# Meeso1/nmmo

Hardware: AMD Instinct MI355X
Metric: agent-steps/sec (whole node), 128-agent envs at 1/2/4/8 MI355X (higher is better)
Workload: dtype int16

## Files before the change

nmmo_amd/csrc/agent_obs.h:

```cpp
#pragma once

#include <utility>

#include "kernels.h"
#include "wire.h"

namespace nmmo {

#ifndef NMMO_AO_WAVES
#define NMMO_AO_WAVES 4
#define NMMO_AO_AGENTS 16
#endif
constexpr int kAoWaves = NMMO_AO_WAVES;
constexpr int kAoAgents = NMMO_AO_AGENTS;
constexpr int kAoRows = kMaxSlots / 64;
constexpr uint32_t kAoEmpty = 0xFFFFFFFFu;
static_assert(kSize <= 256 && kMaxSlots <= 2 * 256 && kMaxSlots % 64 == 0, "packed entity word; two slots per thread (>= 256 threads)");
__host__ __device__ inline int ao_stride(int S) { return ((S + 1) >> 1 | 1) << 1; }
__host__ __device__ inline size_t ao_entity_lds(int S) {
  return (((size_t)NMMO_N_ENTITY_COLS * ao_stride(S) * 2 + 15) & ~(size_t)15) + (size_t)(kMaxSlots + 64) * 4;
}
__host__ __device__ inline uint32_t ao_pack(int slot, int row, int col, bool immune, bool danger, bool player) {
  return (uint32_t)(row & 255) | (uint32_t)(slot & 255) << 8 | (uint32_t)(col & 255) << 16 | (uint32_t)(slot >> 8) << 24 |
         (immune ? 1u << 25 : 0u) | (danger ? 1u << 26 : 0u) | (player ? 1u << 27 : 0u);
}
__device__ __forceinline__ int ao_slot(uint32_t w) { return (int)(((w >> 8) & 255u) | ((w >> 16) & 256u)); }
__device__ __forceinline__ int ao_row(uint32_t w) { return (int)(w & 255u); }
__device__ __forceinline__ int ao_col(uint32_t w) { return (int)((w >> 16) & 255u); }
__device__ __forceinline__ bool ao_immune(uint32_t w) { return (w >> 25) & 1u; }
__device__ __forceinline__ bool ao_danger(uint32_t w) { return (w >> 26) & 1u; }
__device__ __forceinline__ bool ao_player(uint32_t w) { return (w >> 27) & 1u; }
typedef unsigned short ao_u16x2 __attribute__((ext_vector_type(2)));
__device__ __forceinline__ bool ao_in_window(uint32_t w, uint32_t rc) {
  ao_u16x2 d = __builtin_bit_cast(ao_u16x2, w & 0x00FF00FFu) - __builtin_bit_cast(ao_u16x2, rc) +
               (ao_u16x2){(unsigned short)kVision, (unsigned short)kVision};
  return (d.x > d.y ? d.x : d.y) <= 2 * kVision;
}
static_assert(kMaxSlots <= 512 && kSize <= 255, "packed entity word");

constexpr int kSecN[12] = {3, 101, NMMO_MARKET_ROWS + 1, kInv + 1, kInv + 1, kNObs + 1, 99, kNObs + 1, 5, kInv + 1, 99, kInv + 1};
__host__ __device__ constexpr int sec_flat(int k) { return k == 0 ? 0 : sec_flat(k - 1) + kSecN[k - 1]; }
__host__ __device__ constexpr int sec_wire(int k) { return k < 2 ? sec_flat(k) : sec_flat(k) - kWireBuyN; }
static_assert(sec_flat(2) == kWireBuyLo && sec_flat(12) == kMaskN && sec_flat(1) == kMkAttackT &&
                  sec_flat(3) == kMkDestroy && sec_flat(4) == kMkGiveI && sec_flat(5) == kMkGiveT &&
                  sec_flat(6) == kMkGoldP && sec_flat(7) == kMkGoldT && sec_flat(8) == kMkMove &&
                  sec_flat(9) == kMkSellI && sec_flat(10) == kMkSellP && sec_flat(11) == kMkUse,
              "sections (wire.h)");
__host__ inline bool ao_layout_ok(const ObsParams& p) {
  const int offs[12] = {p.o_style, p.o_target, p.o_buy, p.o_destroy, p.o_give_item, p.o_give_target,
                        p.o_gg_price, p.o_gg_target, p.o_move, p.o_sell_item, p.o_sell_price, p.o_use};
  for (int k = 0; k < 12; k++)
    if (offs[k] != sec_flat(k)) return false;
  return p.o_agent_id == sec_flat(12);
}

__device__ __forceinline__ int ao_lane() {
  int l = (int)(threadIdx.x & 63u);
  asm volatile("" : "+v"(l));
  return l;
}

__device__ __forceinline__ uint64_t low_bits(int n) { return n >= 64 ? ~0ull : n <= 0 ? 0ull : (1ull << n) - 1ull; }
template <int L>
__device__ __forceinline__ int writelane(int v, int x) {
  static_assert(L >= 0 && L < 64, "lane");
  int sv = __builtin_amdgcn_readfirstlane(v);
  asm volatile("" : "+s"(sv));
  asm volatile("v_writelane_b32 %0, %1, %2" : "+v"(x) : "s"(sv), "n"(L));
  return x;
}
template <int kLane0, int kIdx0, int... D>
__device__ __forceinline__ int writelanes_(const uint32_t* img, int x, std::integer_sequence<int, D...>) {
  ((x = writelane<kLane0 + D>((int)img[kIdx0 + D], x)), ...);
  return x;
}
template <int kLane0, int kIdx0, int kN>
__device__ __forceinline__ int writelanes(const uint32_t* img, int x) {
  return writelanes_<kLane0, kIdx0>(img, x, std::make_integer_sequence<int, kN>{});
}

template <int kOff, int kN, int kW>
__device__ __forceinline__ void put_field(uint32_t (&img)[kW], uint64_t lo, uint64_t hi) {
  static_assert((kOff + kN + 31) / 32 <= kW, "image size");
#pragma unroll
  for (int d = kOff / 32; d <= (kOff + kN - 1) / 32; d++) {
    const int st = 32 * d - kOff;
    uint32_t x;
    if (st < 0) x = (uint32_t)(lo << (-st));
    else if (st == 0) x = (uint32_t)lo;
    else if (st < 64) x = (uint32_t)((lo >> st) | (hi << (64 - st)));
    else x = (uint32_t)(hi >> (st - 64));
    img[d] |= x;
  }
}

constexpr int kAoStageIt = (NMMO_N_ENTITY_COLS * (kMaxSlots / 8) + 255) / 256;
struct AoStage {
  uint4 x[kAoStageIt];
  int al[2], ds[2];
  int nm, mv;
};
__device__ __forceinline__ void ao_stage_load(const ObsParams& p, int e, AoStage& r) {
  const int S = p.S, tid = threadIdx.x;
  const int16_t* E = p.ent + (size_t)e * NMMO_NF * S;
  const int w4 = S / 8;
  const int nw = NMMO_N_ENTITY_COLS * w4;
  r.nm = p.mcount[e];
  r.mv = p.mlist[(size_t)e * NMMO_MARKET_ROWS + min(tid, NMMO_MARKET_ROWS - 1)];
#pragma unroll
  for (int k = 0; k < kAoStageIt; k++) {
    const int i = tid + (int)blockDim.x * k;
    const int f = i / w4, j = i - f * w4;
    r.x[k] = i < nw ? reinterpret_cast<const uint4*>(E + (size_t)f * S)[j] : make_uint4(0u, 0u, 0u, 0u);
  }
#pragma unroll
  for (int u = 0; u < 2; u++) {
    const int s = min(tid + (int)blockDim.x * u, S - 1);
    r.al[u] = E[F_ALIVE * S + s];
    r.ds[u] = E[F_DS_ROW * S + s];
  }
}
__device__ __forceinline__ void ao_stage_store(const ObsParams& p, int e, int16_t* T, uint32_t* pk, const AoStage& r) {
  const int S = p.S, P = p.P, Sp = ao_stride(S), tid = threadIdx.x;
  const int16_t* E = p.ent + (size_t)e * NMMO_NF * S;
  const int w4 = S / 8;
  const int nw = NMMO_N_ENTITY_COLS * w4;
  constexpr int kIt = kAoStageIt;
  const int(&al)[2] = r.al;
  const int(&ds)[2] = r.ds;
#pragma unroll
  for (int k = 0; k < kIt; k++) {
    const int i = tid + (int)blockDim.x * k;
    if (i < nw) {
      const int f = i / w4, j = i - f * w4;
      uint32_t* d = reinterpret_cast<uint32_t*>(T + f * Sp) + 4 * j;
      d[0] = r.x[k].x;
      d[1] = r.x[k].y;
      d[2] = r.x[k].z;
      d[3] = r.x[k].w;
    }
  }
  for (int i = tid + (int)blockDim.x * kIt; i < nw; i += blockDim.x) {
    const int f = i / w4, j = i - f * w4;
    const uint4 y = reinterpret_cast<const uint4*>(E + (size_t)f * S)[j];
    uint32_t* d = reinterpret_cast<uint32_t*>(T + f * Sp) + 4 * j;
    d[0] = y.x;
    d[1] = y.y;
    d[2] = y.z;
    d[3] = y.w;
  }
  for (int k = tid; k < kMaxSlots + 64; k += blockDim.x) pk[k] = kAoEmpty;
  __syncthreads();
#pragma unroll
  for (int u = 0; u < 2; u++) {
    const int s = tid + (int)blockDim.x * u;
    if (s < S && al[u] && (unsigned)(ds[u] - 1) < (unsigned)S) {
      const bool player = s < P;
      const bool immune = player && T[F_TIME_ALIVE * Sp + s] < p.spawn_immunity;
      const bool danger = T[F_NPC_TYPE * Sp + s] > 1;
      pk[ds[u] - 1] = ao_pack(s, T[F_ROW * Sp + s], T[F_COL * Sp + s], immune, danger, player);
    }
  }
  __syncthreads();
}
__device__ __forceinline__ uint2 ao_listing_load(const ObsParams& p, int e, const AoStage& r) {
  const int own = min((r.mv >> 16) & 255, p.P - 1), slot = min((r.mv >> 24) & 15, kInv - 1);
  return p.items[((size_t)e * p.P + own) * kInv + slot];
}

__device__ __forceinline__ void ao_env_group(int n_envs, int G, int& e, int& g) {
  const int id = blockIdx.x;
  if ((n_envs & 7) == 0) {
    const int x = id & 7, q = id >> 3;
    g = q % G;
    e = (q / G) * 8 + x;
  } else {
    e = id / G;
    g = id - e * G;
  }
}

constexpr int kAoWinRowBytes = 20;
constexpr int kAoWinAgentBytes = 15 * kAoWinRowBytes;
__host__ __device__ inline size_t ao_win_lds(int agents = kAoAgents) {
  return (size_t)agents * kAoWinAgentBytes + (size_t)agents * kInv * 8;
}
__device__ __forceinline__ int ao_clamp_pos(int x) { return min(max(x, kVision), kSize - 1 - kVision); }
struct AoNoop {
  __device__ void operator()() const {}
};
template <int kAgents = kAoAgents, typename F = AoNoop>
__device__ inline void ao_stage_windows(const ObsParams& p, int e, int g, const int16_t* T, int Sp, uint32_t* ws, uint2* is,
                                        F before_barrier = F()) {
  const int tid = threadIdx.x, P = p.P;
  const int la = tid / 15, row = tid - 15 * la, a = g * kAgents + la;
  const bool win = tid < kAgents * 15 && a < P;
  uint32_t d[5] = {0u, 0u, 0u, 0u, 0u};
  if (win) {
    const int r = ao_clamp_pos(T[F_ROW * Sp + a]), c = ao_clamp_pos(T[F_COL * Sp + a]);
    const int base = (r - kVision + row) * kSize + c - kVision;
    const uint32_t* src = reinterpret_cast<const uint32_t*>(p.mat + (size_t)e * kTiles) + (base >> 2);
#pragma unroll
    for (int k = 0; k < 5; k++) d[k] = src[k];
  }
  uint2 iw = make_uint2(0u, 0u);
  const bool itm = tid < kAgents * kInv && g * kAgents + tid / kInv < P;
  if (itm) iw = p.items[((size_t)e * P + g * kAgents) * kInv + tid];
  if (win) {
#pragma unroll
    for (int k = 0; k < 5; k++) ws[tid * 5 + k] = d[k];
  }
  if (tid < kAgents * kInv) is[tid] = iw;
  before_barrier();
  __syncthreads();
}
__device__ __forceinline__ void ao_win_offsets(int (&wo)[2]) {
  wo[0] = wo[1] = 0;
#pragma unroll
  for (int i = 0; i < 4; i++) {
    const int t = lane_id() + 64 * i;
    const int o = t < 225 ? (t / 15) * kAoWinRowBytes + t % 15 : 0;
    wo[i >> 1] |= o << (16 * (i & 1));
  }
}
__device__ __forceinline__ int ao_win_off(const int (&wo)[2], int i) { return (wo[i >> 1] >> (16 * (i & 1))) & 0xFFFF; }

__device__ __forceinline__ int ao_compact(const uint32_t (&pr)[kAoRows], int S, int r, int c, uint32_t* visw) {
  int nvis = 0;
  const uint32_t rc = (uint32_t)r | (uint32_t)c << 16;
#pragma unroll
  for (int i = 0; i < kAoRows; i++) {
    if (64 * i >= S) break;
    const uint32_t x = pr[i];
    const bool in = ao_in_window(x, rc);
    const uint64_t b = __ballot(in);
    const int pos = nvis + __popcll(b & lanes_below());
    if (in && pos < kNObs) visw[pos] = x;
    nvis += __popcll(b);
  }
  return nvis;
}

__device__ __forceinline__ void ao_window_offsets(int (&mo)[2]) {
  mo[0] = mo[1] = 0;
#pragma unroll
  for (int i = 0; i < 4; i++) {
    const int t = lane_id() + 64 * i;
    const int o = t < 225 ? (t / 15 - kVision) * kSize + t % 15 - kVision : 0;
    mo[i >> 1] |= (o & 0xFFFF) << (16 * (i & 1));
  }
}
__device__ __forceinline__ int ao_window_off(const int (&mo)[2], int i) {
  return (int)(int16_t)(uint16_t)((uint32_t)mo[i >> 1] >> (16 * (i & 1)));
}

__device__ __forceinline__ uint32_t ao_move_bits(uint32_t wm1) {
  uint32_t b = 0u;
#pragma unroll
  for (int d = 0; d < 5; d++) {
    const int t = (kVision + dir_dr(d)) * 15 + kVision + dir_dc(d);
    if (!impassable((int)__builtin_amdgcn_readlane((int)wm1, t - 64))) b |= 1u << d;
  }
  return b;
}

static_assert(F_ALCHEMY_LEVEL == F_MELEE_LEVEL + 14 && F_FISHING_LEVEL == F_MELEE_LEVEL + 6 &&
                  F_HERBALISM_LEVEL == F_MELEE_LEVEL + 8, "skill level fields");
__host__ __device__ constexpr uint64_t ao_req_lut() {
  uint64_t m = 0;
  for (int t = 0; t < 16; t++) {
    const int k = (t >= T_SPEAR && t <= T_WAND) ? t - T_SPEAR : (t >= T_WHETSTONE && t <= T_RUNES) ? t - T_WHETSTONE
                  : (t >= T_ROD && t <= T_CHISEL) ? 3 + t - T_ROD : 8;
    m |= (uint64_t)k << (4 * t);
  }
  return m;
}
static_assert(T_RATION == 16 && T_POTION == 17, "requirement table: ration -> fishing, potion -> herbalism");
__device__ __forceinline__ uint64_t ao_usable_ballot(const int16_t* T, int Sp, int ti, uint2 it, bool have) {
  const int lane = ao_lane();
  int lv = 0;
  if (lane < 8) {
    lv = T[(F_MELEE_LEVEL + 2 * lane) * Sp + ti];
  } else if (lane == 8) {
    lv = max((int)T[F_MELEE_LEVEL * Sp + ti], max((int)T[F_RANGE_LEVEL * Sp + ti], (int)T[F_MAGE_LEVEL * Sp + ti]));
  }
  const int type = it_type(it);
  const int k = type < 16 ? (int)((ao_req_lut() >> (4 * type)) & 15u) : type == T_RATION ? 3 : type == T_POTION ? 4 : 8;
  const int req = __shfl(lv, k);
  const bool eq = type >= T_HAT && type <= T_RUNES && it_equipped(it);
  return __ballot(have && !it_price(it) && (eq || it_level(it) <= req));
}

struct AoSections {
  uint64_t s0, s1[2], s3, s4, s5[2], s6[2], s7[2], s8, s9, s10[2], s11;
};
struct AoAgent {
  int a, ti, r, c, gold, aid, nv, ninv, prev_price;
  uint32_t mv;
};
template <bool kWrap>
__device__ __forceinline__ AoSections ao_sections(const ObsParams& p, const int16_t* T, int Sp, const uint32_t* visw,
                                                 const AoAgent& g, uint2 it) {
  const bool combat = (p.systems & NMMO_SYS_COMBAT) != 0;
  const bool item = (p.systems & NMMO_SYS_ITEM) != 0;
  const bool exch = item && (p.systems & NMMO_SYS_EXCHANGE) != 0;
  const bool no_give = kWrap && (p.wflags & kWrapObsNoGive);
  const bool no_danger = kWrap && (p.wflags & kWrapObsNoDangerous);
  const int lane = ao_lane();
  AoSections x;
  x.s1[0] = x.s1[1] = x.s5[0] = x.s5[1] = x.s7[0] = x.s7[1] = 0ull;
#pragma unroll
  for (int h = 0; h < 2; h++) {
    if (64 * h >= g.nv) break;
    const int k = 64 * h + lane;
    bool tgt = false, st = false;
    if (k < g.nv) {
      const uint32_t w = visw[k];
      const int q = ao_slot(w);
      tgt = combat && q != g.a && linf(g.r, g.c, ao_row(w), ao_col(w)) <= 3 && !ao_immune(w) &&
            !(no_danger && ao_danger(w));
      st = ao_player(w) && q != g.a && ao_row(w) == g.r && ao_col(w) == g.c;
    }
    x.s1[h] = __ballot(tgt);
    const uint64_t sb = __ballot(st);
    if (item && !no_give) x.s5[h] = sb;
    if (exch && !no_give) x.s7[h] = sb;
  }
  x.s1[1] |= 1ull << (kNObs - 64);
  x.s5[1] |= 1ull << (kNObs - 64);
  x.s7[1] |= 1ull << (kNObs - 64);
  const bool have = lane < g.ninv;
  const bool fr = have && !it_equipped(it) && !it_price(it);
  const uint64_t bfr = __ballot(fr);
  x.s3 = (item ? bfr : 0ull) | 1ull << kInv;
  x.s4 = (item && !no_give ? bfr : 0ull) | 1ull << kInv;
  x.s9 = (exch ? __ballot(have && !it_equipped(it)) : 0ull) | 1ull << kInv;
  x.s11 = (item ? ao_usable_ballot(T, Sp, g.ti, it, have) : 0ull) | 1ull << kInv;
  x.s0 = combat ? low_bits(kSecN[0]) : 0ull;
  x.s6[0] = x.s6[1] = x.s10[0] = x.s10[1] = 0ull;
  if (exch) {
    const int ng = no_give ? min(g.gold, 1) : min(g.gold, kSecN[6]);
    x.s6[0] = low_bits(ng);
    x.s6[1] = low_bits(ng - 64);
    x.s10[0] = low_bits(kSecN[10]);
    x.s10[1] = low_bits(kSecN[10] - 64);
    if constexpr (kWrap) {
      const int pp = g.prev_price;
      if ((p.wflags & kWrapObsPrice) && pp >= 0 && pp < kSecN[10]) {
        const uint64_t clr = ~(1ull << (pp & 63));
        if (pp < 64) x.s10[0] &= clr;
        else x.s10[1] &= clr;
      }
    }
  }
  x.s8 = g.mv;
  return x;
}

template <bool kFlat, int kW>
__device__ __forceinline__ void ao_image(const AoSections& x, uint32_t (&img)[kW]) {
#pragma unroll
  for (int d = 0; d < kW; d++) img[d] = 0u;
#define AO_PUT(k, lo, hi) put_field<kFlat ? sec_flat(k) : sec_wire(k), kSecN[k], kW>(img, lo, hi)
  AO_PUT(0, x.s0, 0ull);
  AO_PUT(1, x.s1[0], x.s1[1]);
  AO_PUT(3, x.s3, 0ull);
  AO_PUT(4, x.s4, 0ull);
  AO_PUT(5, x.s5[0], x.s5[1]);
  AO_PUT(6, x.s6[0], x.s6[1]);
  AO_PUT(7, x.s7[0], x.s7[1]);
  AO_PUT(8, x.s8, 0ull);
  AO_PUT(9, x.s9, 0ull);
  AO_PUT(10, x.s10[0], x.s10[1]);
  AO_PUT(11, x.s11, 0ull);
#undef AO_PUT
}

}
```

nmmo_amd/csrc/flat_obs.hip:

```cpp
#include "agent_obs.h"

namespace nmmo {

#ifndef NMMO_FO_ABL
#define NMMO_FO_ABL 0
#endif
#ifndef NMMO_FO_STAMPS
#define NMMO_FO_STAMPS 0
#endif
#if NMMO_FO_STAMPS
constexpr int kFoStamps = 12;
__device__ uint64_t fo_stamp_buf[1 << 17][kFoStamps];
__device__ uint64_t fo_wave_buf[1 << 15][6];
#define FO_STAMP(k) fst[k] = __builtin_amdgcn_s_memtime()
#else
#define FO_STAMP(k) (void)0
#endif
#ifndef NMMO_FO_XCD
#define NMMO_FO_XCD 1
#endif
#ifndef NMMO_FO_TILE_SKIP
#define NMMO_FO_TILE_SKIP 0
#endif
#ifndef NMMO_FO_TASK_BATCH
#define NMMO_FO_TASK_BATCH 8
#endif
constexpr int kFoTaskBatch = NMMO_FO_TASK_BATCH;
constexpr int kFoStagedListings = 256;
constexpr int kFoChunks = 25;
static_assert(kFoChunks * 64 >= kMaskN + 2 && (kFoChunks - 1) * 64 < kMaskN, "mask chunks");
static_assert(sec_flat(2) == 104 && sec_flat(3) == 104 + NMMO_MARKET_ROWS + 1, "Buy.MarketItem bits");
constexpr int kFoBuyLo = sec_flat(2);
constexpr int kFoId = kMaskN, kFoEntity = kFoId + 2, kFoInv = kFoEntity + kNObs * NMMO_N_ENTITY_COLS,
              kFoMarket = kFoInv + kInv * 16, kFoTask = kFoMarket + NMMO_MARKET_ROWS * 16;

__host__ __device__ inline size_t fo_lds_bytes(int S) {
  return ao_entity_lds(S) + (size_t)NMMO_MARKET_ROWS * 2 + (size_t)kFoStagedListings * 8 +
         (size_t)kAoWaves * 128 * 4 + ao_win_lds();
}

template <int kSh>
__device__ __forceinline__ uint64_t fo_shift(uint64_t lo, uint64_t hi) {
  if constexpr (kSh >= 64) {
    return 0ull;
  } else if constexpr (kSh > 0) {
    return lo << kSh;
  } else if constexpr (kSh == 0) {
    return lo;
  } else if constexpr (-kSh < 64) {
    return (lo >> (-kSh)) | (hi << (64 + kSh));
  } else if constexpr (-kSh < 128) {
    return hi >> (-kSh - 64);
  } else {
    return 0ull;
  }
}
template <int kK, int kC>
__device__ __forceinline__ uint64_t fo_sec(uint64_t lo, uint64_t hi) {
  constexpr int off = sec_flat(kK), n = kSecN[kK];
  if constexpr (off >= 64 * kC + 64 || off + n <= 64 * kC) return 0ull;
  else return fo_shift<off - 64 * kC>(lo, hi);
}
template <int kC>
__device__ __forceinline__ uint64_t fo_chunk(const AoSections& x) {
  return fo_sec<0, kC>(x.s0, 0ull) | fo_sec<1, kC>(x.s1[0], x.s1[1]) | fo_sec<3, kC>(x.s3, 0ull) |
         fo_sec<4, kC>(x.s4, 0ull) | fo_sec<5, kC>(x.s5[0], x.s5[1]) | fo_sec<6, kC>(x.s6[0], x.s6[1]) |
         fo_sec<7, kC>(x.s7[0], x.s7[1]) | fo_sec<8, kC>(x.s8, 0ull) | fo_sec<9, kC>(x.s9, 0ull) |
         fo_sec<10, kC>(x.s10[0], x.s10[1]) | fo_sec<11, kC>(x.s11, 0ull);
}
__device__ __forceinline__ float fo_bit(uint64_t m) { return __builtin_amdgcn_inverse_ballot_w64(m) ? 1.f : 0.f; }
__device__ __forceinline__ void fo_st(float* row, uint32_t idx, float v) {
  *reinterpret_cast<float*>(reinterpret_cast<char*>(row) + (idx << 2)) = v;
}

constexpr int kFoTail0 = (kFoBuyLo + NMMO_MARKET_ROWS) / 64;
__host__ __device__ constexpr int fo_slot(int c) { return c < 2 ? c : c - kFoTail0 + 2; }
static_assert(fo_slot(kFoChunks - 1) == 9 && kZext == 10 + 1 + 12, "tracked chunks | position | items");
struct FoImg {
  bool ext;
  uint32_t lo, hi;
  int j10;
  int nimg;
  int nst;
};
__device__ __forceinline__ uint64_t fo_prev(const FoImg& g, int slot) {
  return (uint64_t)(uint32_t)__builtin_amdgcn_readlane((int)g.lo, g.j10 + slot) |
         (uint64_t)(uint32_t)__builtin_amdgcn_readlane((int)g.hi, g.j10 + slot) << 32;
}
template <int kC>
__device__ __forceinline__ void fo_put(float* row, FoImg& g, uint64_t m, float aid, float tick) {
  constexpr int sl = fo_slot(kC);
  const int lane = ao_lane();
  const bool same = g.ext && m == fo_prev(g, sl);
  if constexpr (kC == kFoChunks - 1) {
    constexpr int n = kMaskN - 64 * kC;
    if (!same) {
      if (lane < n + 2) fo_st(row, 64 * kC + lane, lane < n ? fo_bit(m) : lane == n ? aid : tick);
      g.nst += n + 2;
    } else {
      if (lane == n + 1) fo_st(row, 64 * kC + lane, tick);
      g.nst += 1;
    }
  } else if (!same) {
    fo_st(row, 64 * kC + lane, fo_bit(m));
    g.nst += 64;
  }
  g.nimg = writelane<2 * sl>((int)(uint32_t)m, g.nimg);
  g.nimg = writelane<2 * sl + 1>((int)(uint32_t)(m >> 32), g.nimg);
}
template <int kC>
__device__ __forceinline__ void fo_tail_chunks(float* row, FoImg& g, const AoSections& x, uint64_t buy17, float aid,
                                               float tick) {
  if constexpr (kC < kFoChunks) {
    uint64_t m = fo_chunk<kC>(x);
    if constexpr (kC == kFoTail0) m |= buy17 | 1ull << ((kFoBuyLo + NMMO_MARKET_ROWS) & 63);
    fo_put<kC>(row, g, m, aid, tick);
    fo_tail_chunks<kC + 1>(row, g, x, buy17, aid, tick);
  }
}

struct IcDesc {
  uint32_t tmA, tmB;
  uint32_t f;
};
__device__ __forceinline__ IcDesc ic_desc(int col) {
  auto bits = [](int lo, int hi) { return ((2u << hi) - 1u) & ~((1u << lo) - 1u); };
  IcDesc d{0u, 0u, 0u};
  auto bf = [&](int sel, int sh, int wd) { d.f = (uint32_t)(sel | sh << 1 | wd << 6); };
  switch (col) {
    case 0: bf(1, 16, 16); break;
    case 1: bf(0, 0, 5); break;
    case 2: d.f = 1u << 11; break;
    case 3: bf(0, 5, 4); break;
    case 5: bf(1, 0, 16); break;
    case 6: case 7: case 8:
      d.tmA = 1u << (T_SPEAR + col - 6) | 1u << (T_WHETSTONE + col - 6);
      d.f = 5u << 12 | 5u << 20;
      break;
    case 9: case 10: case 11:
      d.tmA = bits(T_HAT, T_BOTTOM);
      d.tmB = bits(T_ROD, T_CHISEL);
      d.f = 3u << 12 | 2u << 16;
      break;
    case 12: d.tmA = 1u << T_POTION; d.f = 5u << 12 | 50u << 20; break;
    case 13: d.tmA = 1u << T_RATION; d.f = 5u << 12 | 50u << 20; break;
    case 14: bf(0, 9, 1); break;
    case 15: bf(0, 10, 7); break;
    default: break;
  }
  return d;
}
__device__ __forceinline__ float ic_value(uint2 w, int owner, const IcDesc& d) {
  const int type = (int)(w.x & 31u), lvl = (int)((w.x >> 5) & 15u);
  const uint32_t bfv = __builtin_amdgcn_ubfe((d.f & 1u) ? w.y : w.x, (d.f >> 1) & 31u, (d.f >> 6) & 31u);
  const int ta = (int)((d.tmA >> type) & 1u), tb = (int)((d.tmB >> type) & 1u);
  const int mult = ta * (int)((d.f >> 12) & 15u) + tb * (int)((d.f >> 16) & 15u);
  return (float)((int)bfv + (int)((d.f >> 11) & 1u) * owner + mult * lvl + ((ta | tb) ? (int)(d.f >> 20) : 0));
}
static_assert(T_POTION < 32 && T_RATION < 32 && T_WHETSTONE + 2 < 32, "item type masks");

__device__ __forceinline__ int fo_compact(const uint32_t (&pr)[kAoRows], int r, int c, uint32_t* visw) {
  int nvis = 0;
  const uint32_t rc = (uint32_t)r | (uint32_t)c << 16;
#pragma unroll
  for (int i = 0; i < kAoRows; i++) {
    const bool in = ao_in_window(pr[i], rc);
    const uint64_t b = __ballot(in);
    const int pos = nvis + __popcll(b & lanes_below());
    if (in && pos < kNObs) visw[pos] = pr[i];
    nvis += __popcll(b);
  }
  return nvis;
}

typedef const __attribute__((address_space(4))) ObsParams* FoArgs;

template <bool kWrap, int kS>
__global__ void __launch_bounds__(64 * kAoWaves) flat_obs_kernel(ObsParams p) {
  extern __shared__ __attribute__((aligned(16))) unsigned char smem[];
  const int S = kS ? kS : p.S, P = p.P, Sp = ao_stride(S), tdim = p.task_dim, elems = kFoTask + tdim + 225 * 3;
  int16_t* T = reinterpret_cast<int16_t*>(smem);
  uint32_t* pk = reinterpret_cast<uint32_t*>(smem + ao_entity_lds(S) - (size_t)(kMaxSlots + 64) * 4);
  uint16_t* mpo = reinterpret_cast<uint16_t*>(pk + kMaxSlots + 64);
  uint2* mitem = reinterpret_cast<uint2*>(mpo + NMMO_MARKET_ROWS);
  uint32_t* visw_all = reinterpret_cast<uint32_t*>(mitem + kFoStagedListings);
  uint32_t* wst = visw_all + kAoWaves * 128;
  uint2* ist = reinterpret_cast<uint2*>(wst + kAoAgents * kAoWinAgentBytes / 4);
#if NMMO_FO_XCD
  int el, g;
  ao_env_group(p.env_list ? p.n_list : p.n_envs, (p.P + kAoAgents - 1) / kAoAgents, el, g);
#else
  const int el = blockIdx.x, g = blockIdx.y;
#endif
  const int e = p.env_list ? p.env_list[el] : el, tid = threadIdx.x, lane = lane_id();
  if ((unsigned)e >= (unsigned)p.n_envs) return;
  if (NMMO_FO_ABL & 128) return;
#if NMMO_FO_STAMPS
  uint64_t wst_[6];
  wst_[0] = __builtin_amdgcn_s_memtime();
#endif
  const int w = __builtin_amdgcn_readfirstlane(wave_id());
  AoStage sg;
  ao_stage_load(p, e, sg);
  const int16_t* E = p.ent + (size_t)e * NMMO_NF * S;
  constexpr int kPerWave = kAoAgents / kAoWaves;
  const int abase = g * kAoAgents + w;
  int my_task = 0, my_prev = -1, my_alive = 0;
  uint64_t my_z = 0, my_s = 0;
  const bool mine = lane < kPerWave && abase + kAoWaves * lane < P;
  {
    const int aj = min(abase + kAoWaves * min(lane, kPerWave - 1), P - 1);
    const size_t ai = (size_t)e * P + aj;
    my_task = p.assign[ai];
    my_alive = E[F_ALIVE * S + aj];
    if (p.zrow) {
      my_z = p.zrow[ai];
      my_s = p.zst[ai];
    }
    if constexpr (kWrap)
      if (p.ws) my_prev = p.ws[ai].prev_price;
  }
  ao_stage_store(p, e, T, pk, sg);
  if (!mine) {
    my_task = 0, my_prev = -1, my_alive = 0;
    my_z = my_s = 0;
  }
#if NMMO_FO_STAMPS
  wst_[1] = __builtin_amdgcn_s_memtime();
#endif

  uint32_t pr[kAoRows];
#pragma unroll
  for (int i = 0; i < kAoRows; i++) pr[i] = pk[lane + 64 * i];
  uint32_t* visw = visw_all + w * 128;
  const uint8_t* wsb = reinterpret_cast<const uint8_t*>(wst);
  const float tickf = (float)p.env[(size_t)e * NMMO_NE + E_TICK];
  const bool exch = (p.systems & NMMO_SYS_ITEM) && (p.systems & NMMO_SYS_EXCHANGE);

  const bool zvl = p.ztag && my_z == p.ztag;
  const bool zzl = zvl && (my_s & kZsZero);
  const uint64_t zvalid = __ballot(zvl), zzero = __ballot(zzl), ztask = __ballot(zvl && !zzl && zs_task(my_s) == my_task);
  const uint64_t zextv = __ballot(zvl && !zzl && (my_s & kZsExt));
  const uint64_t ztile = __ballot(zvl && (my_s & kZsTile));
  uint2 img = make_uint2(0u, 0u), pinv = make_uint2(0u, 0u);
  const int ja = lane < 40 ? lane / 10 : lane - 40, ji = lane / 12;
  const bool img_ok = lane < 44 && abase + kAoWaves * ja < P && ((zextv >> ja) & 1);
  const bool pinv_ok = lane < 48 && abase + kAoWaves * ji < P && ((zextv >> ji) & 1);
  if (p.zext) {
    const int aa = min(abase + kAoWaves * min(ja, kPerWave - 1), P - 1);
    const int ai = min(abase + kAoWaves * min(ji, kPerWave - 1), P - 1);
    img = reinterpret_cast<const uint2*>(p.zext)[((size_t)e * P + aa) * kZext + (lane < 40 ? lane % 10 : 10)];
    pinv = reinterpret_cast<const uint2*>(p.zext)[((size_t)e * P + ai) * kZext + 11 + min(lane, 47) % 12];
  }
  const int nm = min(max(sg.nm, 0), NMMO_MARKET_ROWS);
  const uint2 lwd = ao_listing_load(p, e, sg);
  ao_stage_windows(p, e, g, T, Sp, wst, ist, [&]() {
    if (tid < nm) {
      mpo[tid] = (uint16_t)(it_price(lwd) | ((sg.mv >> 16) & 255) << 8);
      if (tid < kFoStagedListings) mitem[tid] = lwd;
    }
    for (int j = tid + (int)blockDim.x; j < nm; j += blockDim.x) {
      const int v = p.mlist[(size_t)e * NMMO_MARKET_ROWS + j];
      const int own = (v >> 16) & 255, slot = (v >> 24) & 15;
      const uint2 wd = p.items[((size_t)e * P + own) * kInv + slot];
      mpo[j] = (uint16_t)(it_price(wd) | own << 8);
      if (j < kFoStagedListings) mitem[j] = wd;
    }
  });
#if NMMO_FO_STAMPS
  wst_[2] = __builtin_amdgcn_s_memtime();
#endif
  asm volatile("" : "+v"(img.x), "+v"(img.y), "+v"(pinv.x), "+v"(pinv.y), "+v"(my_prev));
  if (!img_ok) img = make_uint2(0u, 0u);
  if (!pinv_ok) pinv = make_uint2(0u, 0u);
  const int my_h = !zvl ? (kNObs | NMMO_MARKET_ROWS << 12) : zzl ? 0 : (zs_hv(my_s) | zs_hm(my_s) << 12);
  int nrows = 0;
  unsigned long long nbytes = 0;
  int wo[2];
  ao_win_offsets(wo);
  int toff[4];
#pragma unroll
  for (int i = 0; i < 4; i++) {
    const int t = lane + 64 * i;
    toff[i] = ((t / 15 - kVision) & 255) | (t % 15 - kVision) * 256;
  }
  const int ef = lane & 31, eh = lane >> 5;
  const int iq = lane >> 4;
  const IcDesc icd = ic_desc(lane & 15);

#if NMMO_FO_STAMPS
  wst_[3] = __builtin_amdgcn_s_memtime();
#endif
#pragma unroll 1
  for (int j = 0; j < ((NMMO_FO_ABL & 64) ? 0 : kPerWave); j++) {
    const int a = abase + kAoWaves * j;
    if (a >= P) break;
    const int lane = ao_lane();
    FoArgs kp = (FoArgs)__builtin_amdgcn_kernarg_segment_ptr();
    asm volatile("" : "+s"(kp));
    auto grow = (__attribute__((address_space(1))) float*)(p.obs + ((NMMO_FO_ABL & 256)
        ? (size_t)(((e * P + a) & 15) + 16 * (blockIdx.x & 7)) : (size_t)e * P + a) * elems);
    asm volatile("" : "+s"(grow));
    float* row = (float*)grow;
    const bool zv = (zvalid >> j) & 1;
    const int hj = __builtin_amdgcn_readlane(my_h, j);
    const int hv = hj & 4095, hm = hj >> 12;
    if (!__builtin_amdgcn_readlane(my_alive, j)) {
      if ((zzero >> j) & 1) {
        if ((ztile >> j) & 1) {
          wave_zero(row, kFoTask + tdim, elems);
          nbytes += 4ull * (elems - kFoTask - tdim);
          if (lane == 0) kp->zst[(size_t)e * P + a] = kZsZero;
          nrows++;
        }
        continue;
      }
      if (zv) {
        wave_zero(row, 0, kFoEntity + hv * NMMO_N_ENTITY_COLS);
        wave_zero(row, kFoInv, kFoMarket + hm * 16);
        wave_zero(row, kFoTask, elems);
        nbytes += 4ull * (kFoEntity + hv * NMMO_N_ENTITY_COLS + kFoMarket + hm * 16 - kFoInv + elems - kFoTask);
      } else {
        wave_zero(row, 0, elems);
        nbytes += 4ull * elems;
      }
      if (lane == 0) {
        kp->zrow[(size_t)e * P + a] = kp->ztag;
        kp->zst[(size_t)e * P + a] = kZsZero;
      }
      nrows++;
      continue;
    }
    nrows++;
#if NMMO_FO_STAMPS
    uint64_t fst[kFoStamps];
#endif
    FO_STAMP(0);
    const int la = a - g * kAoAgents;
    const int r = __builtin_amdgcn_readfirstlane(T[F_ROW * Sp + a]);
    const int c = __builtin_amdgcn_readfirstlane(T[F_COL * Sp + a]);
    const int gold = __builtin_amdgcn_readfirstlane(T[F_GOLD * Sp + a]);
    const int aid = __builtin_amdgcn_readfirstlane(T[F_ID * Sp + a]);
    const uint8_t* wa = wsb + la * kAoWinAgentBytes + ((c - kVision) & 3);
    uint32_t wm[4];
#pragma unroll
    for (int i = 0; i < 4; i++) wm[i] = lane + 64 * i < 225 ? wa[ao_win_off(wo, i)] : 0u;
    const uint2 it = lane < kInv ? ist[la * kInv + lane] : make_uint2(0u, 0u);
    const uint32_t mv = ao_move_bits(wm[1]);
    const int ninv = __builtin_ctzll(~__ballot(lane < kInv && it_type(it) != 0));
    const int nv = (NMMO_FO_ABL & 32) ? 0 : min(fo_compact(pr, r, c, visw), kNObs);
    __builtin_amdgcn_fence(__ATOMIC_RELEASE, "wavefront");
    __builtin_amdgcn_wave_barrier();
    __builtin_amdgcn_fence(__ATOMIC_ACQUIRE, "wavefront");

    FO_STAMP(1);
    const bool ext = (zextv >> j) & 1;
    FoImg fg{ext, img.x, img.y, 10 * j, 0, 0};
    if (!(NMMO_FO_ABL & 1)) {
      AoAgent ag;
      ag.a = a;
      ag.ti = a;
      ag.r = r;
      ag.c = c;
      ag.gold = gold;
      ag.aid = aid;
      ag.nv = nv;
      ag.ninv = ninv;
      ag.prev_price = kWrap ? __builtin_amdgcn_readlane(my_prev, j) : -1;
      ag.mv = mv;
      const AoSections x = ao_sections<kWrap>(p, T, Sp, visw, ag, it);
      FO_STAMP(2);
      fg.ext = ext;
      fo_put<0>(row, fg, fo_chunk<0>(x), 0.f, 0.f);
      auto buy_word = [&](int m) {
        const int k = 64 * m + lane;
        bool bv = false;
        if (exch && k < nm) {
          const uint32_t po = mpo[k];
          bv = (int)(po & 255u) <= gold && (int)(po >> 8) != a;
        }
        return __ballot(bv);
      };
      const int nbuy = max(nm, hm);
      const int clast = max(1, min((kFoBuyLo + nbuy - 1) >> 6, 16));
      uint64_t bprev = nm > 0 ? buy_word(0) : 0ull;
      fo_put<1>(row, fg, fo_chunk<1>(x) | bprev << (kFoBuyLo & 63), 0.f, 0.f);
      FO_STAMP(3);
#pragma unroll 1
      for (int cc = 2; cc <= clast; cc++) {
        const uint64_t bcur = 64 * (cc - 1) < nm ? buy_word(cc - 1) : 0ull;
        fo_st(row, 64 * cc + lane, fo_bit(bcur << (kFoBuyLo & 63) | bprev >> (64 - (kFoBuyLo & 63))));
        bprev = bcur;
      }
      FO_STAMP(4);
      const uint64_t buy17 = nm > 15 * 64 ? bprev >> (64 - (kFoBuyLo & 63)) : 0ull;
      fo_tail_chunks<kFoTail0>(row, fg, x, buy17, (float)aid, tickf);
      nbytes += 4ull * (fg.nst + 64 * (clast - 1));
    }
    FO_STAMP(5);
    const int nv2 = (nv + 1) & ~1;
    if (!(NMMO_FO_ABL & 2)) {
      const uint32_t de = kFoEntity + (lane - eh);
#pragma unroll 1
      for (int k0 = 0; k0 < nv2; k0 += 2) {
        const int k = k0 + eh;
        if (ef < NMMO_N_ENTITY_COLS)
          fo_st(row, de + k0 * NMMO_N_ENTITY_COLS, k < nv ? (float)T[ef * Sp + ao_slot(visw[k])] : 0.f);
      }
      const int hz = max(nv2, hv);
      wave_zero(row, kFoEntity + nv2 * NMMO_N_ENTITY_COLS, kFoEntity + hz * NMMO_N_ENTITY_COLS);
      nbytes += 4ull * (hz * NMMO_N_ENTITY_COLS + max(nm, hm) * 16);
    }
    FO_STAMP(6);
    const int jl = (12 * j + lane) & 63;
    const uint32_t px = (uint32_t)__shfl((int)pinv.x, jl), py = (uint32_t)__shfl((int)pinv.y, jl);
    const bool inv_same = ext && __ballot(lane < kInv && (px != it.x || py != it.y)) == 0ull;
    if (!inv_same) {
#pragma unroll
      for (int h = 0; h < ((NMMO_FO_ABL & 4) ? 0 : kInv * 16 / 64); h++) {
        const int q = 4 * h + iq;
        float v = 0.f;
        if (4 * h < ninv && q < ninv) v = ic_value(ist[la * kInv + q], aid, icd);
        fo_st(row, kFoInv + 64 * h + lane, v);
      }
      nbytes += 4ull * kInv * 16;
    }
    FO_STAMP(7);
    const int nms = (NMMO_FO_ABL & 8) ? 0 : min(nm, kFoStagedListings);
    for (int k = lane; k < nms * 16; k += 64) fo_st(row, kFoMarket + k, ic_value(mitem[k >> 4], (mpo[k >> 4] >> 8) + 1, icd));
    if (nm > nms && !(NMMO_FO_ABL & 8)) {
      for (int k = nms * 16 + lane; k < nm * 16; k += 64) {
        const int q = k >> 4;
        const int v = kp->mlist[(size_t)e * NMMO_MARKET_ROWS + q];
        const uint2 wd = kp->items[((size_t)e * P + ((v >> 16) & 255)) * kInv + ((v >> 24) & 15)];
        fo_st(row, kFoMarket + k, ic_value(wd, (mpo[q] >> 8) + 1, icd));
      }
    }
    wave_zero(row, kFoMarket + nm * 16, kFoMarket + max(nm, hm) * 16);
    FO_STAMP(8);
    const int task = __builtin_amdgcn_readlane(my_task, j);
    if (!((ztask >> j) & 1)) {
      const float* temb = kp->task + (size_t)task * tdim;
      int k0 = 0;
      for (; k0 + kFoTaskBatch * 64 <= tdim; k0 += kFoTaskBatch * 64) {
        float t[kFoTaskBatch];
#pragma unroll
        for (int i = 0; i < kFoTaskBatch; i++) t[i] = temb[k0 + 64 * i + lane];
#pragma unroll
        for (int i = 0; i < kFoTaskBatch; i++) fo_st(row, kFoTask + k0 + 64 * i + lane, t[i]);
      }
      for (int k = k0 + lane; k < tdim; k += 64) fo_st(row, kFoTask + k, temb[k]);
      nbytes += 4ull * tdim;
    }
    FO_STAMP(9);
    const uint32_t ppos = (uint32_t)__builtin_amdgcn_readlane((int)img.x, 40 + j);
    const bool tkn = NMMO_FO_TILE_SKIP && ext && !((ztile >> j) & 1);
    const bool same_r = tkn && (int)(ppos & 255u) == r, same_c = tkn && (int)((ppos >> 8) & 255u) == c;
    if (!(NMMO_FO_ABL & 16)) {
      float* dt = row + kFoTask + tdim + 3 * lane;
#pragma unroll
      for (int i = 0; i < 4; i++) {
        if (lane + 64 * i < 225) {
          const float vr = (float)(r + ((toff[i] << 24) >> 24)), vc = (float)(c + (toff[i] >> 8)), vm = (float)wm[i];
          if (NMMO_FO_TILE_SKIP) {
            if (!same_r) dt[192 * i] = vr;
            if (!same_c) dt[192 * i + 1] = vc;
            dt[192 * i + 2] = vm;
          } else {
            typedef float f3 __attribute__((ext_vector_type(3)));
            const f3 v = {vr, vc, vm};
            __builtin_memcpy(dt + 192 * i, &v, 12);
          }
        }
      }
      nbytes += 4ull * 225 * (1 + !same_r + !same_c);
    }
    FO_STAMP(10);
    {
      uint32_t* zx = reinterpret_cast<uint32_t*>(kp->zext + ((size_t)e * P + a) * kZext);
      int wv = fg.nimg;
      if (lane == 20) wv = r | c << 8;
      if (lane == 21) wv = 0;
      if (lane < 22) zx[lane] = (uint32_t)wv;
      if (!inv_same && lane < kInv) reinterpret_cast<uint2*>(zx + 22)[lane] = it;
      if (lane == 0) {
        if (!zv) kp->zrow[(size_t)e * P + a] = kp->ztag;
        kp->zst[(size_t)e * P + a] = zs_pack(nv2, nm, task) | kZsExt;
      }
    }
#if NMMO_FO_STAMPS
    FO_STAMP(11);
    if (lane == 0 && (size_t)e * P + a < (1u << 17))
      for (int k = 0; k < kFoStamps; k++) fo_stamp_buf[(size_t)e * P + a][k] = fst[k];
#endif
    __builtin_amdgcn_fence(__ATOMIC_RELEASE, "wavefront");
    __builtin_amdgcn_wave_barrier();
    __builtin_amdgcn_fence(__ATOMIC_ACQUIRE, "wavefront");
  }
#if NMMO_FO_STAMPS
  wst_[4] = __builtin_amdgcn_s_memtime();
  wst_[5] = (uint64_t)e | (uint64_t)nrows << 32;
  {
    const size_t wi = ((size_t)blockIdx.y * gridDim.x + blockIdx.x) * kAoWaves + w;
    if (lane == 0 && wi < (1u << 15))
      for (int k = 0; k < 6; k++) fo_wave_buf[wi][k] = wst_[k];
  }
#endif
  if (p.rows_out && lane == 0 && nrows) {
    atomicAdd(&p.rows_out[2 * e], (unsigned long long)nrows);
    atomicAdd(&p.rows_out[2 * e + 1], nbytes);
  }
}

bool flat_obs_ok(const ObsParams& p) {
  return p.S % 8 == 0 && p.S <= kMaxSlots && p.P <= 128 && p.obs && p.ztag && p.zrow && ao_layout_ok(p) &&
         p.o_agent_id == kFoId && p.o_tick == kFoId + 1 && p.o_entity == kFoEntity && p.o_inventory == kFoInv &&
         p.o_market == kFoMarket && p.o_task == kFoTask && p.o_tile == kFoTask + p.task_dim &&
         p.elems == p.o_tile + 225 * 3;
}

hipError_t launch_flat_obs(const ObsParams& p, hipStream_t stream) {
  if (!flat_obs_ok(p)) return hipErrorInvalidValue;
  const int ne = list_grid(p.env_list, p.n_list, p.n_envs);
  if (ne <= 0) return hipSuccess;
#if NMMO_FO_XCD
  const dim3 grid(ne * ((p.P + kAoAgents - 1) / kAoAgents)), block(64 * kAoWaves);
#else
  const dim3 grid(ne, (p.P + kAoAgents - 1) / kAoAgents), block(64 * kAoWaves);
#endif
  const size_t lds = fo_lds_bytes(p.S);
  if (p.S == kMaxSlots) {
    if (p.wflags) hipLaunchKernelGGL((flat_obs_kernel<true, kMaxSlots>), grid, block, lds, stream, p);
    else hipLaunchKernelGGL((flat_obs_kernel<false, kMaxSlots>), grid, block, lds, stream, p);
  } else {
    if (p.wflags) hipLaunchKernelGGL((flat_obs_kernel<true, 0>), grid, block, lds, stream, p);
    else hipLaunchKernelGGL((flat_obs_kernel<false, 0>), grid, block, lds, stream, p);
  }
  return hipGetLastError();
}

}

#if NMMO_FO_STAMPS
extern "C" __attribute__((visibility("default"))) int nmmo_debug_fo_stamps(void* host, size_t bytes) {
  if (bytes > sizeof(nmmo::fo_stamp_buf)) bytes = sizeof(nmmo::fo_stamp_buf);
  if (hipDeviceSynchronize() != hipSuccess) return -1;
  if (hipMemcpyFromSymbol(host, HIP_SYMBOL(nmmo::fo_stamp_buf), bytes) != hipSuccess) return -1;
  void* d = nullptr;
  if (hipGetSymbolAddress(&d, HIP_SYMBOL(nmmo::fo_stamp_buf)) != hipSuccess) return -1;
  return hipMemset(d, 0, sizeof(nmmo::fo_stamp_buf)) == hipSuccess && hipDeviceSynchronize() == hipSuccess ? 0 : -1;
}
extern "C" __attribute__((visibility("default"))) int nmmo_debug_fo_wave_stamps(void* host, size_t bytes) {
  if (bytes > sizeof(nmmo::fo_wave_buf)) bytes = sizeof(nmmo::fo_wave_buf);
  if (hipDeviceSynchronize() != hipSuccess) return -1;
  if (hipMemcpyFromSymbol(host, HIP_SYMBOL(nmmo::fo_wave_buf), bytes) != hipSuccess) return -1;
  void* d = nullptr;
  if (hipGetSymbolAddress(&d, HIP_SYMBOL(nmmo::fo_wave_buf)) != hipSuccess) return -1;
  return hipMemset(d, 0, sizeof(nmmo::fo_wave_buf)) == hipSuccess && hipDeviceSynchronize() == hipSuccess ? 0 : -1;
}
#endif
```

Baseline: 329.6 million.

## Shrink flat_obs LDS footprint with aliased regions to fit five workgroups per CU

Repacks the flat observation kernel's shared memory so more workgroups fit per CU. The packed entity words now alias the window staging area, and item staging can reuse the row/col columns of T. Market listings share one pool, filled from the top, and the number staged adapts to the listing count. Window rows are realigned to 4 dwords with alignbyte, row/col are read from the packed entity word instead of T, and the kernel requests 5 waves per EU. The aliasing needs an extra barrier before the staging writes, and a smaller static listing staging area can push more market reads to global memory.

```diff
diff --git a/nmmo_amd/csrc/agent_obs.h b/nmmo_amd/csrc/agent_obs.h
--- a/nmmo_amd/csrc/agent_obs.h
+++ b/nmmo_amd/csrc/agent_obs.h
@@ -16,10 +16,12 @@
 constexpr int kAoRows = kMaxSlots / 64;
 constexpr uint32_t kAoEmpty = 0xFFFFFFFFu;
 static_assert(kSize <= 256 && kMaxSlots <= 2 * 256 && kMaxSlots % 64 == 0, "packed entity word; two slots per thread (>= 256 threads)");
-__host__ __device__ inline int ao_stride(int S) { return ((S + 1) >> 1 | 1) << 1; }
-__host__ __device__ inline size_t ao_entity_lds(int S) {
-  return (((size_t)NMMO_N_ENTITY_COLS * ao_stride(S) * 2 + 15) & ~(size_t)15) + (size_t)(kMaxSlots + 64) * 4;
-}
+__host__ __device__ constexpr int ao_stride(int S) { return ((S + 1) >> 1 | 1) << 1; }
+__host__ __device__ constexpr size_t ao_columns_lds(int S) {
+  return ((size_t)NMMO_N_ENTITY_COLS * ao_stride(S) * 2 + 15) & ~(size_t)15;
+}
+constexpr size_t kAoPkBytes = (size_t)(kMaxSlots + 64) * 4;
+__host__ __device__ constexpr size_t ao_entity_lds(int S) { return ao_columns_lds(S) + kAoPkBytes; }
 __host__ __device__ inline uint32_t ao_pack(int slot, int row, int col, bool immune, bool danger, bool player) {
   return (uint32_t)(row & 255) | (uint32_t)(slot & 255) << 8 | (uint32_t)(col & 255) << 16 | (uint32_t)(slot >> 8) << 24 |
          (immune ? 1u << 25 : 0u) | (danger ? 1u << 26 : 0u) | (player ? 1u << 27 : 0u);
@@ -182,16 +184,17 @@
 
 constexpr int kAoWinRowBytes = 20;
 constexpr int kAoWinAgentBytes = 15 * kAoWinRowBytes;
-__host__ __device__ inline size_t ao_win_lds(int agents = kAoAgents) {
+__host__ __device__ constexpr size_t ao_win_lds(int agents = kAoAgents) {
   return (size_t)agents * kAoWinAgentBytes + (size_t)agents * kInv * 8;
 }
 __device__ __forceinline__ int ao_clamp_pos(int x) { return min(max(x, kVision), kSize - 1 - kVision); }
 struct AoNoop {
   __device__ void operator()() const {}
 };
-template <int kAgents = kAoAgents, typename F = AoNoop>
+template <int kAgents = kAoAgents, int kRowDw = kAoWinRowBytes / 4, typename F = AoNoop, typename B = AoNoop>
 __device__ inline void ao_stage_windows(const ObsParams& p, int e, int g, const int16_t* T, int Sp, uint32_t* ws, uint2* is,
-                                        F before_barrier = F()) {
+                                        F before_barrier = F(), B before_writes = B()) {
+  static_assert(kRowDw == 4 || kRowDw == 5, "window row: 5 aligned dwords, or 4 realigned");
   const int tid = threadIdx.x, P = p.P;
   const int la = tid / 15, row = tid - 15 * la, a = g * kAgents + la;
   const bool win = tid < kAgents * 15 && a < P;
@@ -202,24 +205,30 @@
     const uint32_t* src = reinterpret_cast<const uint32_t*>(p.mat + (size_t)e * kTiles) + (base >> 2);
 #pragma unroll
     for (int k = 0; k < 5; k++) d[k] = src[k];
+    if constexpr (kRowDw == 4) {
+#pragma unroll
+      for (int k = 0; k < 4; k++) d[k] = __builtin_amdgcn_alignbyte(d[k + 1], d[k], (uint32_t)(c - kVision) & 3u);
+    }
   }
   uint2 iw = make_uint2(0u, 0u);
   const bool itm = tid < kAgents * kInv && g * kAgents + tid / kInv < P;
   if (itm) iw = p.items[((size_t)e * P + g * kAgents) * kInv + tid];
+  before_writes();
   if (win) {
 #pragma unroll
-    for (int k = 0; k < 5; k++) ws[tid * 5 + k] = d[k];
+    for (int k = 0; k < kRowDw; k++) ws[tid * kRowDw + k] = d[k];
   }
   if (tid < kAgents * kInv) is[tid] = iw;
   before_barrier();
   __syncthreads();
 }
+template <int kRowBytes = kAoWinRowBytes>
 __device__ __forceinline__ void ao_win_offsets(int (&wo)[2]) {
   wo[0] = wo[1] = 0;
 #pragma unroll
   for (int i = 0; i < 4; i++) {
     const int t = lane_id() + 64 * i;
-    const int o = t < 225 ? (t / 15) * kAoWinRowBytes + t % 15 : 0;
+    const int o = t < 225 ? (t / 15) * kRowBytes + t % 15 : 0;
     wo[i >> 1] |= o << (16 * (i & 1));
   }
 }
diff --git a/nmmo_amd/csrc/flat_obs.hip b/nmmo_amd/csrc/flat_obs.hip
--- a/nmmo_amd/csrc/flat_obs.hip
+++ b/nmmo_amd/csrc/flat_obs.hip
@@ -26,7 +26,7 @@
 #define NMMO_FO_TASK_BATCH 8
 #endif
 constexpr int kFoTaskBatch = NMMO_FO_TASK_BATCH;
-constexpr int kFoStagedListings = 256;
+constexpr int kFoStagedListings = 64;
 constexpr int kFoChunks = 25;
 static_assert(kFoChunks * 64 >= kMaskN + 2 && (kFoChunks - 1) * 64 < kMaskN, "mask chunks");
 static_assert(sec_flat(2) == 104 && sec_flat(3) == 104 + NMMO_MARKET_ROWS + 1, "Buy.MarketItem bits");
@@ -34,10 +34,28 @@
 constexpr int kFoId = kMaskN, kFoEntity = kFoId + 2, kFoInv = kFoEntity + kNObs * NMMO_N_ENTITY_COLS,
               kFoMarket = kFoInv + kInv * 16, kFoTask = kFoMarket + NMMO_MARKET_ROWS * 16;
 
-__host__ __device__ inline size_t fo_lds_bytes(int S) {
-  return ao_entity_lds(S) + (size_t)NMMO_MARKET_ROWS * 2 + (size_t)kFoStagedListings * 8 +
-         (size_t)kAoWaves * 128 * 4 + ao_win_lds();
-}
+constexpr int kFoVisw = (kNObs + 3) & ~3;
+constexpr int kFoWinRowBytes = 16, kFoWinAgentBytes = 15 * kFoWinRowBytes;
+constexpr size_t kFoWinBytes = (size_t)kAoAgents * kFoWinAgentBytes, kFoItemBytes = (size_t)kAoAgents * kInv * 8;
+static_assert(F_COL == F_ROW + 1 && kAoPkBytes <= kFoWinBytes, "shared LDS regions");
+__host__ __device__ constexpr bool fo_items_in_T(int S) {
+  return (size_t)2 * ao_stride(S) * 2 >= kFoItemBytes && (F_ROW * ao_stride(S) * 2) % 8 == 0;
+}
+constexpr int kFoListPool = NMMO_MARKET_ROWS * 2 + kFoStagedListings * 8;
+__host__ __device__ constexpr int fo_staged(int nm) {
+  return nm < ((kFoListPool - ((2 * nm + 7) & ~7)) >> 3) ? nm : (kFoListPool - ((2 * nm + 7) & ~7)) >> 3;
+}
+static_assert(fo_staged(NMMO_MARKET_ROWS) == kFoStagedListings && fo_staged(256) == 256 && fo_staged(257) == 255 &&
+                  fo_staged(0) == 0 && kFoListPool % 16 == 0, "listings' pool");
+__host__ __device__ constexpr size_t fo_lds_bytes(int S) {
+  return ao_columns_lds(S) + (size_t)kFoListPool +
+         (size_t)kAoWaves * kFoVisw * 4 + kFoWinBytes + (fo_items_in_T(S) ? 0 : kFoItemBytes);
+}
+constexpr size_t kFoLdsGranule = 1280;
+static_assert(kAoAgents != 16 ||
+                  (5 * fo_lds_bytes(kMaxSlots) <= 160 * 1024 && fo_items_in_T(kMaxSlots) &&
+                   5 * ((fo_lds_bytes(kMaxSlots) + kFoLdsGranule - 1) / kFoLdsGranule * kFoLdsGranule) <= 160 * 1024),
+              "5 workgroups per CU");
 
 template <int kSh>
 __device__ __forceinline__ uint64_t fo_shift(uint64_t lo, uint64_t hi) {
@@ -176,16 +194,17 @@
 typedef const __attribute__((address_space(4))) ObsParams* FoArgs;
 
 template <bool kWrap, int kS>
-__global__ void __launch_bounds__(64 * kAoWaves) flat_obs_kernel(ObsParams p) {
+__global__ void __launch_bounds__(64 * kAoWaves) __attribute__((amdgpu_waves_per_eu(5, 5))) flat_obs_kernel(ObsParams p) {
   extern __shared__ __attribute__((aligned(16))) unsigned char smem[];
   const int S = kS ? kS : p.S, P = p.P, Sp = ao_stride(S), tdim = p.task_dim, elems = kFoTask + tdim + 225 * 3;
   int16_t* T = reinterpret_cast<int16_t*>(smem);
-  uint32_t* pk = reinterpret_cast<uint32_t*>(smem + ao_entity_lds(S) - (size_t)(kMaxSlots + 64) * 4);
-  uint16_t* mpo = reinterpret_cast<uint16_t*>(pk + kMaxSlots + 64);
-  uint2* mitem = reinterpret_cast<uint2*>(mpo + NMMO_MARKET_ROWS);
-  uint32_t* visw_all = reinterpret_cast<uint32_t*>(mitem + kFoStagedListings);
-  uint32_t* wst = visw_all + kAoWaves * 128;
-  uint2* ist = reinterpret_cast<uint2*>(wst + kAoAgents * kAoWinAgentBytes / 4);
+  uint16_t* mpo = reinterpret_cast<uint16_t*>(smem + ao_columns_lds(S));
+  uint32_t* visw_all = reinterpret_cast<uint32_t*>(mpo) + kFoListPool / 4;
+  uint2* mtop = reinterpret_cast<uint2*>(visw_all) - 1;
+  uint32_t* wst = visw_all + kAoWaves * kFoVisw;
+  uint32_t* pk = wst;
+  uint2* ist = reinterpret_cast<uint2*>(fo_items_in_T(S) ? smem + (size_t)F_ROW * Sp * 2
+                                                         : reinterpret_cast<unsigned char*>(wst) + kFoWinBytes);
 #if NMMO_FO_XCD
   int el, g;
   ao_env_group(p.env_list ? p.n_list : p.n_envs, (p.P + kAoAgents - 1) / kAoAgents, el, g);
@@ -225,6 +244,11 @@
     my_task = 0, my_prev = -1, my_alive = 0;
     my_z = my_s = 0;
   }
+  uint32_t my_rc;
+  {
+    const int aj = min(abase + kAoWaves * min(lane, kPerWave - 1), P - 1);
+    my_rc = (uint32_t)(uint16_t)T[F_ROW * Sp + aj] | (uint32_t)(uint16_t)T[F_COL * Sp + aj] << 16;
+  }
 #if NMMO_FO_STAMPS
   wst_[1] = __builtin_amdgcn_s_memtime();
 #endif
@@ -232,7 +256,7 @@
   uint32_t pr[kAoRows];
 #pragma unroll
   for (int i = 0; i < kAoRows; i++) pr[i] = pk[lane + 64 * i];
-  uint32_t* visw = visw_all + w * 128;
+  uint32_t* visw = visw_all + w * kFoVisw;
   const uint8_t* wsb = reinterpret_cast<const uint8_t*>(wst);
   const float tickf = (float)p.env[(size_t)e * NMMO_NE + E_TICK];
   const bool exch = (p.systems & NMMO_SYS_ITEM) && (p.systems & NMMO_SYS_EXCHANGE);
@@ -252,21 +276,21 @@
     img = reinterpret_cast<const uint2*>(p.zext)[((size_t)e * P + aa) * kZext + (lane < 40 ? lane % 10 : 10)];
     pinv = reinterpret_cast<const uint2*>(p.zext)[((size_t)e * P + ai) * kZext + 11 + min(lane, 47) % 12];
   }
-  const int nm = min(max(sg.nm, 0), NMMO_MARKET_ROWS);
+  const int nm = min(max(sg.nm, 0), NMMO_MARKET_ROWS), nst = fo_staged(nm);
   const uint2 lwd = ao_listing_load(p, e, sg);
-  ao_stage_windows(p, e, g, T, Sp, wst, ist, [&]() {
+  ao_stage_windows<kAoAgents, kFoWinRowBytes / 4>(p, e, g, T, Sp, wst, ist, [&]() {
     if (tid < nm) {
       mpo[tid] = (uint16_t)(it_price(lwd) | ((sg.mv >> 16) & 255) << 8);
-      if (tid < kFoStagedListings) mitem[tid] = lwd;
+      if (tid < nst) mtop[-tid] = lwd;
     }
     for (int j = tid + (int)blockDim.x; j < nm; j += blockDim.x) {
       const int v = p.mlist[(size_t)e * NMMO_MARKET_ROWS + j];
       const int own = (v >> 16) & 255, slot = (v >> 24) & 15;
       const uint2 wd = p.items[((size_t)e * P + own) * kInv + slot];
       mpo[j] = (uint16_t)(it_price(wd) | own << 8);
-      if (j < kFoStagedListings) mitem[j] = wd;
-    }
-  });
+      if (j < nst) mtop[-j] = wd;
+    }
+  }, []() { __syncthreads(); });
 #if NMMO_FO_STAMPS
   wst_[2] = __builtin_amdgcn_s_memtime();
 #endif
@@ -277,7 +301,7 @@
   int nrows = 0;
   unsigned long long nbytes = 0;
   int wo[2];
-  ao_win_offsets(wo);
+  ao_win_offsets<kFoWinRowBytes>(wo);
   int toff[4];
 #pragma unroll
   for (int i = 0; i < 4; i++) {
@@ -337,11 +361,11 @@
 #endif
     FO_STAMP(0);
     const int la = a - g * kAoAgents;
-    const int r = __builtin_amdgcn_readfirstlane(T[F_ROW * Sp + a]);
-    const int c = __builtin_amdgcn_readfirstlane(T[F_COL * Sp + a]);
+    const int rcj = __builtin_amdgcn_readlane((int)my_rc, j);
+    const int r = (int16_t)(rcj & 0xFFFF), c = rcj >> 16;
     const int gold = __builtin_amdgcn_readfirstlane(T[F_GOLD * Sp + a]);
     const int aid = __builtin_amdgcn_readfirstlane(T[F_ID * Sp + a]);
-    const uint8_t* wa = wsb + la * kAoWinAgentBytes + ((c - kVision) & 3);
+    const uint8_t* wa = wsb + la * kFoWinAgentBytes;
     uint32_t wm[4];
 #pragma unroll
     for (int i = 0; i < 4; i++) wm[i] = lane + 64 * i < 225 ? wa[ao_win_off(wo, i)] : 0u;
@@ -401,11 +425,20 @@
     const int nv2 = (nv + 1) & ~1;
     if (!(NMMO_FO_ABL & 2)) {
       const uint32_t de = kFoEntity + (lane - eh);
+      const bool epos = (lane & 31) == F_ROW || (lane & 31) == F_COL;
+      const uint32_t esh = (lane & 31) == F_COL ? 16u : 0u;
 #pragma unroll 1
       for (int k0 = 0; k0 < nv2; k0 += 2) {
         const int k = k0 + eh;
-        if (ef < NMMO_N_ENTITY_COLS)
-          fo_st(row, de + k0 * NMMO_N_ENTITY_COLS, k < nv ? (float)T[ef * Sp + ao_slot(visw[k])] : 0.f);
+        if (ef < NMMO_N_ENTITY_COLS) {
+          float v = 0.f;
+          if (k < nv) {
+            const uint32_t vw = visw[k];
+            const int tv = T[ef * Sp + ao_slot(vw)];
+            v = (float)(epos ? (int)((vw >> esh) & 255u) : tv);
+          }
+          fo_st(row, de + k0 * NMMO_N_ENTITY_COLS, v);
+        }
       }
       const int hz = max(nv2, hv);
       wave_zero(row, kFoEntity + nv2 * NMMO_N_ENTITY_COLS, kFoEntity + hz * NMMO_N_ENTITY_COLS);
@@ -426,8 +459,8 @@
       nbytes += 4ull * kInv * 16;
     }
     FO_STAMP(7);
-    const int nms = (NMMO_FO_ABL & 8) ? 0 : min(nm, kFoStagedListings);
-    for (int k = lane; k < nms * 16; k += 64) fo_st(row, kFoMarket + k, ic_value(mitem[k >> 4], (mpo[k >> 4] >> 8) + 1, icd));
+    const int nms = (NMMO_FO_ABL & 8) ? 0 : fo_staged(nm);
+    for (int k = lane; k < nms * 16; k += 64) fo_st(row, kFoMarket + k, ic_value(mtop[-(k >> 4)], (mpo[k >> 4] >> 8) + 1, icd));
     if (nm > nms && !(NMMO_FO_ABL & 8)) {
       for (int k = nms * 16 + lane; k < nm * 16; k += 64) {
         const int q = k >> 4;
```

Result: faster. 341.2 million (median of 6 runs) (+3.5%).
